# slimgroup/dfno

Hardware: AMD Instinct MI355X
Metric: sec/batch (lower is better)
Workload: dtype fp32; 1 GPU; model=dfno-two-phase-3d, global_batch=1, t_in=1, t_out=30, width=20, num_blocks=4, parallelism=spatial-model-parallel 1x1x1x1x1x1, step=fwd+relative-Lp-loss+bwd+adam, spectral_weights=complex64

## Files before the change

dfno_amd/csrc/adam.hip:

```cpp

#include <hip/hip_runtime.h>
#include <hip/hip_bf16.h>
#include <hip/hip_fp8.h>
#include <torch/extension.h>
#include <ATen/hip/impl/HIPStreamMasqueradingAsCUDA.h>

#include <map>
#include <vector>

#include "kernels.h"
#include "device_util.h"


namespace {

using namespace dfno_io;

constexpr int kBlock = 256;
constexpr long kGridCap = 256L * 8;

template <typename T, bool VECTOR>
__global__ void adam_step_kernel(T* __restrict__ p, const T* __restrict__ g,
                                 T* __restrict__ m, T* __restrict__ v,
                                 long n, T lr, T b1, T b2, T eps, T wd,
                                 T c1, T c2) {
  long i0 = (long)blockIdx.x * blockDim.x + threadIdx.x;
// ... 61 lines not shown
  for (long i = i0; i < total4; i += stride) {
    while (i >= tab.end4[t]) ++t;
    long base = (t == 0) ? 0 : tab.end4[t - 1];
    long j = (i - base) * 4;
    float4 pv = *reinterpret_cast<float4*>(tab.p[t] + j);
    const float4 gv = *reinterpret_cast<const float4*>(tab.g[t] + j);
    float4 mv = *reinterpret_cast<float4*>(tab.m[t] + j);
    float4 vv = *reinterpret_cast<float4*>(tab.v[t] + j);
    float pr[4] = {pv.x, pv.y, pv.z, pv.w};
    float gr[4] = {gv.x, gv.y, gv.z, gv.w};
    float mr[4] = {mv.x, mv.y, mv.z, mv.w};
    float vr[4] = {vv.x, vv.y, vv.z, vv.w};
    const float c1 = tab.c1[t], c2 = tab.c2[t];
#pragma unroll
    for (int k = 0; k < 4; ++k) {
      float gg = gr[k] + wd * pr[k];
      mr[k] = b1 * mr[k] + (1.f - b1) * gg;
      vr[k] = b2 * vr[k] + (1.f - b2) * gg * gg;
      pr[k] -= lr * (mr[k] / c1) / (sqrtf(vr[k] / c2) + eps);
    }
    *reinterpret_cast<float4*>(tab.p[t] + j) = make_float4(pr[0], pr[1], pr[2], pr[3]);
    *reinterpret_cast<float4*>(tab.m[t] + j) = make_float4(mr[0], mr[1], mr[2], mr[3]);
    *reinterpret_cast<float4*>(tab.v[t] + j) = make_float4(vr[0], vr[1], vr[2], vr[3]);
  }
}

struct AdamTabB {
  unsigned short* p[kAdamMaxT];
  const unsigned short* g[kAdamMaxT];
  unsigned short* m[kAdamMaxT];
  unsigned short* v[kAdamMaxT];
  long end8[kAdamMaxT];
  long nn[kAdamMaxT];
  float c1[kAdamMaxT], c2[kAdamMaxT];
// ... 7 lines not shown
  long stride = (long)gridDim.x * blockDim.x;
  int t = 0;
  for (long i = i0; i < total8; i += stride) {
    while (i >= tab.end8[t]) ++t;
    long base = (t == 0) ? 0 : tab.end8[t - 1];
    long j = (i - base) * 8;
    const float c1 = tab.c1[t], c2 = tab.c2[t];
    if (j + 8 <= tab.nn[t]) {
      float pr[8], gr[8], mr[8], vr[8];
      load8(tab.p[t] + j, pr);
      load8(tab.g[t] + j, gr);
      load8(tab.m[t] + j, mr);
      load8(tab.v[t] + j, vr);
#pragma unroll
      for (int k = 0; k < 8; ++k) {
        float gg = gr[k] + wd * pr[k];
        mr[k] = b1 * mr[k] + (1.f - b1) * gg;
        vr[k] = b2 * vr[k] + (1.f - b2) * gg * gg;
        pr[k] -= lr * (mr[k] / c1) / (sqrtf(vr[k] / c2) + eps);
      }
      store8(tab.p[t] + j, pr);
      store8(tab.m[t] + j, mr);
      store8(tab.v[t] + j, vr);
    } else {
      for (long e = j; e < tab.nn[t]; ++e) {
        float pv = __uint_as_float(((unsigned int)tab.p[t][e]) << 16);
        float gv = __uint_as_float(((unsigned int)tab.g[t][e]) << 16);
        float mv = __uint_as_float(((unsigned int)tab.m[t][e]) << 16);
        float vv = __uint_as_float(((unsigned int)tab.v[t][e]) << 16);
        float gg = gv + wd * pv;
        mv = b1 * mv + (1.f - b1) * gg;
        vv = b2 * vv + (1.f - b2) * gg * gg;
        pv -= lr * (mv / c1) / (sqrtf(vv / c2) + eps);
        __hip_bfloat16 hp = __float2bfloat16(pv);
        __hip_bfloat16 hm = __float2bfloat16(mv);
        __hip_bfloat16 hv = __float2bfloat16(vv);
        tab.p[t][e] = *reinterpret_cast<unsigned short*>(&hp);
        tab.m[t][e] = *reinterpret_cast<unsigned short*>(&hm);
        tab.v[t][e] = *reinterpret_cast<unsigned short*>(&hv);
      }
    }
  }
}

template <bool QOUT>
__global__ __launch_bounds__(kBlock) void adam_multi_uniform_kernel(
    AdamTab tab, AdamFp8Tab qt, long n4, float lr, float b1, float b2,
    float eps, float wd) {
// ... 7 lines not shown
  if constexpr (QOUT) inv = 448.f / fmaxf(*qt.am_in[t], 1e-30f);
  long i0 = (long)blockIdx.x * blockDim.x + threadIdx.x;
  long stride = (long)gridDim.x * blockDim.x;
  for (long i = i0; i < n4; i += stride) {
    long j = i * 4;
    float4 pv = *reinterpret_cast<float4*>(p + j);
    const float4 gv = *reinterpret_cast<const float4*>(g + j);
    float4 mv = *reinterpret_cast<float4*>(m + j);
    float4 vv = *reinterpret_cast<float4*>(v + j);
    float pr[4] = {pv.x, pv.y, pv.z, pv.w};
    float gr[4] = {gv.x, gv.y, gv.z, gv.w};
    float mr[4] = {mv.x, mv.y, mv.z, mv.w};
    float vr[4] = {vv.x, vv.y, vv.z, vv.w};
#pragma unroll
    for (int k = 0; k < 4; ++k) {
      float gg = gr[k] + wd * pr[k];
      mr[k] = b1 * mr[k] + (1.f - b1) * gg;
      vr[k] = b2 * vr[k] + (1.f - b2) * gg * gg;
      pr[k] -= lr * (mr[k] / c1) / (sqrtf(vr[k] / c2) + eps);
    }
    *reinterpret_cast<float4*>(p + j) = make_float4(pr[0], pr[1], pr[2], pr[3]);
    *reinterpret_cast<float4*>(m + j) = make_float4(mr[0], mr[1], mr[2], mr[3]);
    *reinterpret_cast<float4*>(v + j) = make_float4(vr[0], vr[1], vr[2], vr[3]);
    if constexpr (QOUT) {
      uchar4 qb;
      __hip_fp8_e4m3 h0(pr[0] * inv), h1(pr[1] * inv), h2(pr[2] * inv),
          h3(pr[3] * inv);
      qb.x = h0.__x; qb.y = h1.__x; qb.z = h2.__x; qb.w = h3.__x;
      *reinterpret_cast<uchar4*>(qt.q[t] + j) = qb;
#pragma unroll
      for (int k = 0; k < 4; ++k) amax = fmaxf(amax, fabsf(pr[k]));
    }
  }
  if constexpr (QOUT) {
// ... 204 lines not shown
```

dfno_amd/csrc/bindings.cpp:

```cpp
#include <torch/extension.h>

#include "kernels.h"

PYBIND11_MODULE(TORCH_EXTENSION_NAME, m) {
  m.doc() = "dfno_amd MI355X (gfx950) native kernels";
  m.def("channel_mix_fwd", &channel_mix_fwd,
        "fused channel linear + bias + gelu: returns (y, z)");
  m.def("channel_mix_fwd_t", &channel_mix_fwd_t,
        "transposed channel contraction (grad-x)");
  m.def("channel_mix_bwd_w", &channel_mix_bwd_w,
        "split-s grad-W (+grad-bias) reduction");
  m.def("linear_res_gelu_fwd", &linear_res_gelu_fwd,
        "fused y = gelu(W @ x + res): returns (y, z)");
  m.def("wide_channel_mix", &wide_channel_mix,
        "MFMA channel mix for 33 <= max(I, O) <= 128 (+bias/res/gelu, "
        "optionally transposed): returns (y, z)");
  m.def("irfft_linear_res_gelu_fwd", &irfft_linear_res_gelu_fwd,
        "fused y = gelu(W @ x + pad_irfft(Yt)): returns (y, z)");
  m.def("rfft_adj_mix", &rfft_adj_mix,
        "fused gx = W^T @ gz + rfft_trunc_adj(G, n)");
  m.def("gelu_fwd", &gelu_fwd, "exact gelu");
  m.def("gelu_bwd", &gelu_bwd, "gelu backward (gy, z) -> gz");
  m.def("add_gelu_fwd", &add_gelu_fwd, "fused residual add + gelu: returns (y, z)");
  m.def("proj_head_fwd", &proj_head_fwd, "fused linear->gelu->linear head");
// ... 25 lines not shown
        "fused padded (z,t) 2-D synthesis (kept-mode c64 -> real)");
  m.def("dft_pad_irfft_bf16", &dft_pad_irfft_bf16,
        "pad_irfft with bf16 output (bf16 compute config)");
  m.def("dft_rfft_trunc_adj_bf16", &dft_rfft_trunc_adj_bf16,
        "rfft_trunc adjoint with bf16 output");
  m.def("spectral_corner_fwd", &spectral_corner_fwd,
        "corner-block complex spectral contraction (accumulate into y box)");
  m.def("spectral_corner_bwd_x", &spectral_corner_bwd_x,
        "corner-block spectral contraction adjoint wrt x");
  m.def("spectral_corners_fwd", &spectral_corners_fwd,
        "all corner boxes in one launch");
  m.def("spectral_corners_bwd_x", &spectral_corners_bwd_x,
        "all corner boxes adjoint wrt x in one launch");
  m.def("spectral_corners_bwd_w", &spectral_corners_bwd_w,
        "multi-corner spectral grad-W (gw[i,o,e] = sum_b x conj(gy))");
  m.def("spectral_corners_fwd_fp8", &spectral_corners_fwd_fp8,
        "fp8-weight spectral contraction (e4m3 packed pairs + per-corner scale)");
  m.def("spectral_corners_bwd_x_fp8", &spectral_corners_bwd_x_fp8,
        "fp8-weight spectral contraction adjoint wrt x");
  m.def("fp8_quant_corners", &fp8_quant_corners,
        "device-side e4m3 requantization of the corner masters");
  m.def("bf16_channel_mix", &bf16_channel_mix,
        "bf16-storage fused channel linear (+bias/res/gelu): returns (y, z)");
  m.def("bf16_channel_mix_bwd_w", &bf16_channel_mix_bwd_w,
        "bf16 grad-W/grad-bias reduction (fp32 accumulation)");
  m.def("bf16_gelu_fwd", &bf16_gelu_fwd, "bf16 exact gelu");
  m.def("bf16_gelu_bwd", &bf16_gelu_bwd, "bf16 gelu backward");
  m.def("bf16_add_gelu", &bf16_add_gelu, "bf16 fused add+gelu: returns (y, z)");
  m.def("pack_boxes", &pack_boxes,
        "gather repartition boxes into one flat staging buffer");
// ... 4 lines not shown
```

dfno_amd/csrc/kernels.h:

```cpp
#pragma once

#include <torch/extension.h>
#define DFNO_CHECK_LAUNCH(what)                                            \
  do {                                                                     \
    hipError_t _e = hipGetLastError();                                     \
    TORCH_CHECK(_e == hipSuccess, what, " launch failed: ",                \
                hipGetErrorString(_e));                                    \
  } while (0)

#include <vector>

std::vector<at::Tensor> channel_mix_fwd(const at::Tensor& x, const at::Tensor& W,
                                        const at::Tensor& b, bool act);

at::Tensor channel_mix_fwd_t(const at::Tensor& gz, const at::Tensor& W);

std::vector<at::Tensor> linear_res_gelu_fwd(const at::Tensor& x, const at::Tensor& W,
                                            const at::Tensor& res);

std::vector<at::Tensor> wide_channel_mix(const at::Tensor& x, const at::Tensor& W,
                                         const at::Tensor& b, const at::Tensor& res,
                                         bool act, bool wt, bool need_z);

std::vector<at::Tensor> irfft_linear_res_gelu_fwd(const at::Tensor& x,
// ... 88 lines not shown
void unpack_boxes(const at::Tensor& flat, at::Tensor& dst,
                  const at::Tensor& desc, int64_t max_numel);

void spectral_corner_fwd(const at::Tensor& x, const at::Tensor& w, at::Tensor& y,
                         std::vector<int64_t> starts);
void spectral_corner_bwd_x(const at::Tensor& gy, const at::Tensor& w, at::Tensor& gx,
                           std::vector<int64_t> starts);

void spectral_corners_fwd(const at::Tensor& x, std::vector<at::Tensor> ws,
                          at::Tensor& y, std::vector<std::vector<int64_t>> starts);
void spectral_corners_bwd_x(const at::Tensor& gy, std::vector<at::Tensor> ws,
                            at::Tensor& gx, std::vector<std::vector<int64_t>> starts);
void spectral_corners_bwd_w(const at::Tensor& x, const at::Tensor& gy,
                            std::vector<at::Tensor> gws,
                            std::vector<std::vector<int64_t>> starts);

void spectral_corners_fwd_fp8(const at::Tensor& x, std::vector<at::Tensor> w16s,
                              std::vector<at::Tensor> amaxes, at::Tensor& y,
                              std::vector<std::vector<int64_t>> starts);
void spectral_corners_bwd_x_fp8(const at::Tensor& gy, std::vector<at::Tensor> w16s,
                                std::vector<at::Tensor> amaxes, at::Tensor& gx,
                                std::vector<std::vector<int64_t>> starts);
void fp8_quant_corners(std::vector<at::Tensor> ws, std::vector<at::Tensor> w16s,
                       std::vector<at::Tensor> amaxes);
```

dfno_amd/csrc/spectral.hip:

```cpp

#include <hip/hip_runtime.h>
#include <hip/hip_fp8.h>
#include <torch/extension.h>
#include <ATen/hip/impl/HIPStreamMasqueradingAsCUDA.h>

#include "kernels.h"
#include "device_util.h"

namespace {

using namespace dfno_io;

constexpr int kBlock = 256;
constexpr int kMaxDims = 6;

struct BoxGeom {
  long box[kMaxDims];
  long fstride[kMaxDims];
  long origin;
  int nd;
  long nelem;
};

template <typename T>
// ... 185 lines not shown
    } else {
      for (int i = 0; i < n_in; ++i) chan(i);
    }

    T* yb = y + 2 * (((long)b * n_out + o0) * Ftot + f);
#pragma unroll
    for (int k = 0; k < OTILE; ++k) {
      if (k < olim) {
        yb[2 * (long)k * Ftot] = accr[k];
        yb[2 * (long)k * Ftot + 1] = acci[k];
      }
    }
  }
}

template <typename T, int ICAP, bool ITILE = false>
__global__ __launch_bounds__(kBlock) void spectral_corners_bwd_w_kernel(
    const T* __restrict__ x, const T* __restrict__ gy, MultiGeom<T> mg,
    int B, int I_, int O, long Ftot) {
  const int ntile = ITILE ? (I_ + ICAP - 1) / ICAP : 1;
  const long total = mg.cum[mg.ncorners] * O * ntile;
  long t0 = (long)blockIdx.x * blockDim.x + threadIdx.x;
  long stride = (long)gridDim.x * blockDim.x;

  for (long t = t0; t < total; t += stride) {
    long work = t % mg.cum[mg.ncorners];
    int o = (int)(t / mg.cum[mg.ncorners]);
    int i0 = 0;
    if (ITILE) { i0 = (o / O) * ICAP; o %= O; }
    const int I = ITILE ? min(ICAP, I_ - i0) : I_;
// ... 15 lines not shown
      for (int k = 0; k < ICAP; ++k) {
        if (k < I) {
          const T xr = xb[2 * (long)k * Ftot], xi = xb[2 * (long)k * Ftot + 1];
          accr[k] += xr * gr + xi * gi;
          acci[k] += xr * gi - xi * gr;
        }
      }
    }
#pragma unroll
    for (int k = 0; k < ICAP; ++k) {
      if (k < I) {
        long widx = 2 * (((long)(i0 + k) * O + o) * g.nelem + e);
        gw[widx] = accr[k];
        gw[widx + 1] = acci[k];
      }
    }
  }
}


BoxGeom make_geom(const at::Tensor& x, const at::Tensor& w,
                  const std::vector<int64_t>& starts) {
  BoxGeom g{};
  int nd = (int)x.dim() - 2;
  TORCH_CHECK(nd >= 1 && nd <= kMaxDims, "spectral: bad ndim");
  TORCH_CHECK((int)w.dim() - 2 == nd, "spectral: w ndim mismatch");
  TORCH_CHECK((int)starts.size() == nd, "spectral: starts size mismatch");
  g.nd = nd;
  g.nelem = 1;
  long stride = 1;
  long fs[kMaxDims];
  for (int d = nd - 1; d >= 0; --d) {
    fs[d] = stride;
    stride *= x.size(d + 2);
  }
  g.origin = 0;
  for (int d = 0; d < nd; ++d) {
    g.box[d] = w.size(d + 2);
    g.fstride[d] = fs[d];
    g.origin += starts[d] * fs[d];
    g.nelem *= g.box[d];
  }
  return g;
}

void check_c(const at::Tensor& t, const char* name) {
  TORCH_CHECK(t.is_cuda(), name, " must be on GPU");
  TORCH_CHECK(t.is_contiguous(), name, " must be contiguous");
  TORCH_CHECK(t.scalar_type() == at::kComplexFloat || t.scalar_type() == at::kComplexDouble,
              name, " must be complex64/complex128");
}

}

void spectral_corner_fwd(const at::Tensor& x, const at::Tensor& w, at::Tensor& y,
                         std::vector<int64_t> starts) {
  check_c(x, "x"); check_c(w, "w"); check_c(y, "y");
  int B = (int)x.size(0), I = (int)x.size(1), O = (int)y.size(1);
  TORCH_CHECK((int)w.size(0) == I && (int)w.size(1) == O, "spectral: w shape");
  long Ftot = 1;
// ... 87 lines not shown
  for (long i = (long)blockIdx.x * blockDim.x + threadIdx.x; i < n;
       i += (long)gridDim.x * blockDim.x) {
    __hip_fp8_e4m3 h(src[i] * inv);
    dst[i] = h.__x;
  }
}

template <typename T, bool CONJT, bool FP8 = false>
static void launch_corners(const at::Tensor& x,
                           const std::vector<at::Tensor>& ws,
                           at::Tensor& y,
                           const std::vector<std::vector<int64_t>>& starts,
                           int B, int I, int O, long Ftot,
                           const std::vector<at::Tensor>* amaxes = nullptr) {
  auto stream = at::hip::getCurrentHIPStreamMasqueradingAsCUDA().stream();
  constexpr int OT = 8;
  const int n_out = CONJT ? I : O;
  long ntiles = (n_out + OT - 1) / OT;

  size_t idx = 0;
  while (idx < ws.size()) {
    MultiGeom<T> mg{};
    mg.ncorners = 0;
    mg.cum[0] = 0;
    while (idx < ws.size() && mg.ncorners < kMaxCorners) {
      BoxGeom g = make_geom(x, ws[idx], starts[idx]);
      if (g.nelem == 0) { ++idx; continue; }
      int c = mg.ncorners++;
      mg.g[c] = g;
      mg.w[c] = reinterpret_cast<const T*>(ws[idx].data_ptr());
      mg.amax[c] = amaxes ? (*amaxes)[idx].data_ptr<float>() : nullptr;
      mg.cum[c + 1] = mg.cum[c] + g.nelem * ntiles;
      ++idx;
    }
    if (mg.ncorners == 0) continue;
    int grid = launch_grid(mg.cum[mg.ncorners] * B, kBlock, 256L * 16);
    const int n_in = CONJT ? O : I;
#define SPC_LAUNCH(NINV)                                                       \
    hipLaunchKernelGGL((spectral_corners_kernel<T, OT, CONJT, NINV, FP8>),     \
                       dim3(grid), dim3(kBlock), 0, stream,                    \
                       reinterpret_cast<const T*>(x.data_ptr()), mg,           \
                       reinterpret_cast<T*>(y.data_ptr()), B, I, O, Ftot);
    if (n_in == 20) { SPC_LAUNCH(20) }
    else if (n_in == 32) { SPC_LAUNCH(32) }
    else if (n_in == 8) { SPC_LAUNCH(8) }
    else { SPC_LAUNCH(0) }
#undef SPC_LAUNCH
  }
}

void spectral_corners_fwd(const at::Tensor& x, std::vector<at::Tensor> ws,
                          at::Tensor& y, std::vector<std::vector<int64_t>> starts) {
// ... 162 lines not shown
  int B = (int)gy.size(0), O = (int)gy.size(1), I = (int)gx.size(1);
  long Ftot = 1;
  for (int d = 2; d < gy.dim(); ++d) Ftot *= gy.size(d);
  for (auto& w : ws) {
    check_c(w, "w");
    TORCH_CHECK((int)w.size(0) == I && (int)w.size(1) == O, "spectral: w shape");
  }
  if (B == 0 || ws.empty()) return;
  if (gy.scalar_type() == at::kComplexFloat) {
    launch_corners<float, true>(gy, ws, gx, starts, B, I, O, Ftot);
  } else {
    launch_corners<double, true>(gy, ws, gx, starts, B, I, O, Ftot);
  }
  DFNO_CHECK_LAUNCH("spectral");
}
```

dfno_amd/nn/block.py:

```python

from __future__ import annotations

import os
from typing import Dict, List, Tuple

import numpy as np
import torch
import torch.nn as nn

from ..comm import (Repartition, _get_plan, repartition_complete,
                    repartition_issue)
from ..partition import Partition, compute_distribution_info
from ..ops import spectral_conv, linear_res_gelu, rfft_trunc, fft_trunc, pad_ifft, pad_irfft
from ..ops import block_epilogue, fused_epilogue_enabled, fused_epilogue_ok
from ..ops.fft import (new_stash_key, rfft_bf16_native_ok, rfft_trunc_stash,
                       stash_fusable, zt_caps_ok, zt_enabled, zt_fwd, zt_inv,
                       zt_native_ok)
from ..timing import comm_region
from .linear import BroadcastedLinear

__all__ = ["DistributedFNOBlock"]


class DistributedFNOBlock(nn.Module):

    def __init__(self, P_x: Partition, in_shape, modes,
                 device=torch.device("cpu"), dtype=torch.float32,
                 spectral_fp8: bool = False):
# ... 70 lines not shown
                if digit == "0":
                    bounds.append((max(0, start) - start, min(mode, stop) - start))
                    gbounds.append((0, mode))
                else:
                    bounds.append((max(dim_size - mode, start) - start,
                                   min(dim_size, stop) - start))
                    gbounds.append((dim_size - mode, dim_size))
            bounds = list(reversed(bounds))
            gbounds = list(reversed(gbounds))
            if any(b - a <= 0 for a, b in bounds):
                continue
            w = nn.Parameter(
                self.scale * torch.rand(self.width, self.width,
                                        *[b - a for a, b in bounds],
                                        device=device, dtype=self.dtype_complex))
            self.weights.append(w)
            self.corner_bounds.append(bounds)
            self.slices.append([slice(None), slice(None)] + [slice(a, b) for a, b in bounds])
            self.corner_ids.append(i)
            self.corner_shapes.append([hi - lo for lo, hi in gbounds])
            loc = []
            for d, (glo, ghi) in zip(range(2, self.P_y.dim), gbounds):
                start, stop = info["start"][d], info["stop"][d]
                loc.append((max(start, glo) - glo, min(stop, ghi) - glo))
            self.corner_local_in_corner.append(loc)

        self.linear = BroadcastedLinear(self.P_x, self.width, self.width,
                                        bias=False, dim=1, device=device, dtype=dtype)

        self.dt_comm = 0.0
# ... 293 lines not shown
```

dfno_amd/ops/spectral.py:

```python

from __future__ import annotations

from typing import List, Sequence, Tuple

import torch

from .. import _ext

__all__ = ["spectral_conv"]


def _corner_slices(bounds: Sequence[Tuple[int, int]]):
    return (slice(None), slice(None)) + tuple(slice(a, b) for a, b in bounds)



_E4M3_MAX = 448.0
_QUANT_EPOCH = [0]
_FP8_CACHE = {}


def bump_quant_epoch() -> None:
    _QUANT_EPOCH[0] += 1
    if _QUANT_EPOCH[0] % 64 == 0:
# ... 25 lines not shown
        for i in range(0, len(stale), 64):
            ext.fp8_quant_corners(stale[i:i + 64], stale16[i:i + 64],
                                  stale_am[i:i + 64])
    out16 = [_FP8_CACHE[id(w)][1] for w in weights]
    amaxes = [_FP8_CACHE[id(w)][2] for w in weights]
    return out16, amaxes


def dequantize_fp8(w16: torch.Tensor, amax) -> torch.Tensor:
    if isinstance(amax, torch.Tensor):
        scale = float(amax.clamp_min(1e-30)) / _E4M3_MAX
    else:
        scale = float(amax)
    w8 = w16.unsqueeze(-1).view(torch.uint8).view(torch.float8_e4m3fn)
    return torch.view_as_complex(w8.to(torch.float32) * scale)


class _SpectralConvFn(torch.autograd.Function):
    @staticmethod
    def forward(ctx, x: torch.Tensor, bounds_list, out_channels: int,
                fp8: bool, *weights: torch.Tensor):
        B, I = x.shape[0], x.shape[1]
        fdims = list(x.shape[2:])
        ctx.fp8 = fp8 = bool(fp8 and x.is_cuda and x.dtype == torch.complex64)
        y = torch.zeros((B, out_channels, *fdims), dtype=x.dtype, device=x.device)
        if fp8 and x.numel() > 0:
            ext = _ext.get(required=True)
            xc = x.contiguous()
            w16s, scales = _fp8_weights(weights)
            ext.spectral_corners_fwd_fp8(
# ... 6 lines not shown
            xc = x.contiguous()
            ext.spectral_corners_fwd(
                xc, [w.contiguous() for w in weights], y,
                [[a for a, _ in bounds] for bounds in bounds_list])
            x_saved = xc
        else:
            if x.is_cuda and x.numel() > 0:
                from ..dispatch import note_fallback
                note_fallback("spectral_conv", f"dtype {x.dtype} not complex64/128")
            x_saved = x
            for w, bounds in zip(weights, bounds_list):
                sl = _corner_slices(bounds)
                y[sl] = torch.einsum("bi...,io...->bo...", x[sl], w)
        ctx.save_for_backward(x_saved, *weights)
        ctx.bounds_list = bounds_list
        return y

    @staticmethod
    def backward(ctx, gy: torch.Tensor):
        x = ctx.saved_tensors[0]
        weights = ctx.saved_tensors[1:]
        bounds_list = ctx.bounds_list
        gy = gy.contiguous()
        gx = torch.zeros_like(x)
        gws = []
        if gy.is_cuda and gy.numel() > 0 and gy.dtype in (torch.complex64, torch.complex128):
            ext = _ext.get(required=True)
            starts = [[a for a, _ in bounds] for bounds in bounds_list]
            if getattr(ctx, "fp8", False):
                w16s, scales = ctx.fp8_wq
                ext.spectral_corners_bwd_x_fp8(gy, w16s, scales, gx, starts)
            else:
                ext.spectral_corners_bwd_x(
                    gy, [w.contiguous() for w in weights], gx, starts)
            if x.shape[1] <= 64:
                gws = [torch.empty_like(w) for w in weights]
                ext.spectral_corners_bwd_w(x.contiguous(), gy, gws, starts)
            else:
                from ..dispatch import note_fallback
                note_fallback("spectral_corners_bwd_w",
                              f"in_channels {x.shape[1]} > 64 (einsum grad-W)")
                for w, bounds in zip(weights, bounds_list):
                    sl = _corner_slices(bounds)
                    gws.append(torch.einsum("bo...,bi...->io...",
                                            gy[sl], x[sl].conj()))
        else:
            for w, bounds in zip(weights, bounds_list):
                sl = _corner_slices(bounds)
                gx[sl] = torch.einsum("bo...,io...->bi...", gy[sl], w.conj())
                gws.append(torch.einsum("bo...,bi...->io...", gy[sl], x[sl].conj()))
        return (gx, None, None, None, *gws)


def spectral_conv(x: torch.Tensor, weights: List[torch.Tensor],
                  bounds_list: List[List[Tuple[int, int]]],
                  out_channels: int = None, fp8: bool = False) -> torch.Tensor:
    if out_channels is None:
        out_channels = weights[0].shape[1] if weights else x.shape[1]
    return _SpectralConvFn.apply(x, bounds_list, out_channels, fp8, *weights)
```

dfno_amd/optim.py:

```python

from __future__ import annotations

import torch

from . import _ext

__all__ = ["Adam"]


class Adam(torch.optim.Adam):

    def __init__(self, *args, **kwargs):
        super().__init__(*args, **kwargs)
        self._flat_cache = {}

    def _flat_views(self, p, state):
        def flat(t):
            r = torch.view_as_real(t) if t.is_complex() else t
            assert r.is_contiguous(), "fused Adam requires contiguous params"
            return r.view(-1)
        ptrs = (p.data_ptr(), state["exp_avg"].data_ptr(),
                state["exp_avg_sq"].data_ptr())
        cached = self._flat_cache.get(id(p))
        if cached is None or cached[0] != ptrs:
            cached = (ptrs, (flat(p), flat(state["exp_avg"]),
                             flat(state["exp_avg_sq"])))
            self._flat_cache[id(p)] = cached
        return cached[1]

    @torch.no_grad()
    def step(self, closure=None):
        loss = None
        if closure is not None:
            with torch.enable_grad():
                loss = closure()

        ext = _ext.get(required=False) if torch.cuda.is_available() else None
        fallback_groups = []
        for group in self.param_groups:
            lr = group["lr"]
            beta1, beta2 = group["betas"]
            eps = group["eps"]
            wd = group["weight_decay"]
            if group.get("amsgrad", False) or ext is None:
                fallback_groups.append(group)
                continue
            slow = []
            batch = ([], [], [], [], [])
            fp8_q, fp8_in, fp8_out, origs = [], [], [], []
            try:
                from .ops.spectral import _FP8_CACHE, _QUANT_EPOCH
            except Exception:
# ... 66 lines not shown
```

training/two_phase/train_two_phase.py:

```python

import argparse
import os
import sys
import time
from pathlib import Path

import numpy as np
import torch

sys.path.insert(0, str(Path(__file__).resolve().parents[2]))

import dfno_amd as dfno
from dfno_amd.data import DistributedSleipnerDataset3D


def main():
    p = argparse.ArgumentParser()
    p.add_argument("--ranks", "-n", type=int, default=None,
                   help="partition size along Y (default: world size)")
    p.add_argument("--data", choices=["synthetic", "local", "azure"], default="synthetic")
    p.add_argument("--data-root", type=str, default=None)
    p.add_argument("--num-train", type=int, default=800)
    p.add_argument("--num-valid", type=int, default=200)
    p.add_argument("--num-epochs", type=int, default=100)
# ... 49 lines not shown
    valid_idx = list(range(args.num_train + 1, args.num_train + args.num_valid + 1))
    mk = lambda idx: DistributedSleipnerDataset3D(
        P_x, idx, client=client, container=container, prefix=prefix,
        shape=shape, normalize=True, savepath=args.cache_dir,
        filename="sample", root=root, synthetic=synthetic)
    train_data, valid_data = mk(train_idx), mk(valid_idx)

    train_loader = torch.utils.data.DataLoader(train_data, batch_size=nb, shuffle=False)
    valid_loader = torch.utils.data.DataLoader(valid_data, batch_size=nb, shuffle=False)
    P_x.barrier()

    model = dfno.DistributedFNONd(
        P_x, [nb, channel_in, *shape[:-1], 1], shape[-1], args.width,
        tuple(args.modes), device=device, dtype=dtype)
    criterion = dfno.DistributedRelativeLpLoss(P_x)
    optimizer = torch.optim.Adam(model.parameters(), lr=args.lr)

    out_dir = Path(args.out_dir)
    if P_root.active:
        out_dir.mkdir(parents=True, exist_ok=True)
    train_accs, valid_accs = [], []

    start_epoch = 0
    if args.resume:
        rdir = Path(args.resume)
        rk = max(P_x.rank, 0)
        cands = sorted(rdir.glob(f"train_state_*_{rk:04d}.pt"))
        if not cands:
            raise FileNotFoundError(
                f"rank {rk}: no train_state_*_{rk:04d}.pt under {rdir}")
        state = torch.load(cands[-1], map_location=device, weights_only=False)
# ... 89 lines not shown
```

Measured before the change: 18.40 ms.

## Fuse spectral grad-W into Adam update and add paired-element spectral contraction kernel

Adds a kernel that computes the spectral corner weight gradient and applies Adam to those weights in the same pass. This is done by deferring grad-W from backward to the optimizer step, so the gradient tensors are never written or read back. It also adds a paired-element spectral contraction path (two frequencies per thread, float4 loads, 4-wide output tiles) for fp32 corners, which can be disabled with an env var. The training script switches to the custom Adam, and the Adam maths moves into a shared helper. The deferral logic brings extra bookkeeping complexity and fallback paths, and it changes when gradients exist.

```diff
diff --git a/dfno_amd/csrc/adam.hip b/dfno_amd/csrc/adam.hip
--- a/dfno_amd/csrc/adam.hip
+++ b/dfno_amd/csrc/adam.hip
@@ -10,6 +10,7 @@
 
 #include "kernels.h"
 #include "device_util.h"
+#include "adam_update.h"
 
 
 namespace {
@@ -101,10 +102,7 @@
     const float c1 = tab.c1[t], c2 = tab.c2[t];
 #pragma unroll
     for (int k = 0; k < 4; ++k) {
-      float gg = gr[k] + wd * pr[k];
-      mr[k] = b1 * mr[k] + (1.f - b1) * gg;
-      vr[k] = b2 * vr[k] + (1.f - b2) * gg * gg;
-      pr[k] -= lr * (mr[k] / c1) / (sqrtf(vr[k] / c2) + eps);
+      adam_update(pr[k], gr[k], mr[k], vr[k], lr, b1, b2, eps, wd, c1, c2);
     }
     *reinterpret_cast<float4*>(tab.p[t] + j) = make_float4(pr[0], pr[1], pr[2], pr[3]);
     *reinterpret_cast<float4*>(tab.m[t] + j) = make_float4(mr[0], mr[1], mr[2], mr[3]);
@@ -142,10 +140,7 @@
       load8(tab.v[t] + j, vr);
 #pragma unroll
       for (int k = 0; k < 8; ++k) {
-        float gg = gr[k] + wd * pr[k];
-        mr[k] = b1 * mr[k] + (1.f - b1) * gg;
-        vr[k] = b2 * vr[k] + (1.f - b2) * gg * gg;
-        pr[k] -= lr * (mr[k] / c1) / (sqrtf(vr[k] / c2) + eps);
+        adam_update(pr[k], gr[k], mr[k], vr[k], lr, b1, b2, eps, wd, c1, c2);
       }
       store8(tab.p[t] + j, pr);
       store8(tab.m[t] + j, mr);
@@ -156,10 +151,7 @@
         float gv = __uint_as_float(((unsigned int)tab.g[t][e]) << 16);
         float mv = __uint_as_float(((unsigned int)tab.m[t][e]) << 16);
         float vv = __uint_as_float(((unsigned int)tab.v[t][e]) << 16);
-        float gg = gv + wd * pv;
-        mv = b1 * mv + (1.f - b1) * gg;
-        vv = b2 * vv + (1.f - b2) * gg * gg;
-        pv -= lr * (mv / c1) / (sqrtf(vv / c2) + eps);
+        adam_update(pv, gv, mv, vv, lr, b1, b2, eps, wd, c1, c2);
         __hip_bfloat16 hp = __float2bfloat16(pv);
         __hip_bfloat16 hm = __float2bfloat16(mv);
         __hip_bfloat16 hv = __float2bfloat16(vv);
@@ -197,10 +189,7 @@
     float vr[4] = {vv.x, vv.y, vv.z, vv.w};
 #pragma unroll
     for (int k = 0; k < 4; ++k) {
-      float gg = gr[k] + wd * pr[k];
-      mr[k] = b1 * mr[k] + (1.f - b1) * gg;
-      vr[k] = b2 * vr[k] + (1.f - b2) * gg * gg;
-      pr[k] -= lr * (mr[k] / c1) / (sqrtf(vr[k] / c2) + eps);
+      adam_update(pr[k], gr[k], mr[k], vr[k], lr, b1, b2, eps, wd, c1, c2);
     }
     *reinterpret_cast<float4*>(p + j) = make_float4(pr[0], pr[1], pr[2], pr[3]);
     *reinterpret_cast<float4*>(m + j) = make_float4(mr[0], mr[1], mr[2], mr[3]);
diff --git a/dfno_amd/csrc/adam_update.h b/dfno_amd/csrc/adam_update.h
--- /dev/null
+++ b/dfno_amd/csrc/adam_update.h
@@ -0,0 +1,13 @@
+#pragma once
+
+#include <hip/hip_runtime.h>
+
+__device__ __forceinline__ void adam_update(float& p, float g, float& m,
+                                            float& v, float lr, float b1,
+                                            float b2, float eps, float wd,
+                                            float c1, float c2) {
+  float gg = g + wd * p;
+  m = b1 * m + (1.f - b1) * gg;
+  v = b2 * v + (1.f - b2) * gg * gg;
+  p -= lr * (m / c1) / (sqrtf(v / c2) + eps);
+}
diff --git a/dfno_amd/csrc/bindings.cpp b/dfno_amd/csrc/bindings.cpp
--- a/dfno_amd/csrc/bindings.cpp
+++ b/dfno_amd/csrc/bindings.cpp
@@ -63,6 +63,8 @@
         "all corner boxes adjoint wrt x in one launch");
   m.def("spectral_corners_bwd_w", &spectral_corners_bwd_w,
         "multi-corner spectral grad-W (gw[i,o,e] = sum_b x conj(gy))");
+  m.def("spectral_gradw_adam_", &spectral_gradw_adam_,
+        "spectral grad-W fused into the Adam update of the corner weights");
   m.def("spectral_corners_fwd_fp8", &spectral_corners_fwd_fp8,
         "fp8-weight spectral contraction (e4m3 packed pairs + per-corner scale)");
   m.def("spectral_corners_bwd_x_fp8", &spectral_corners_bwd_x_fp8,
diff --git a/dfno_amd/csrc/kernels.h b/dfno_amd/csrc/kernels.h
--- a/dfno_amd/csrc/kernels.h
+++ b/dfno_amd/csrc/kernels.h
@@ -126,6 +126,13 @@
 void spectral_corners_bwd_w(const at::Tensor& x, const at::Tensor& gy,
                             std::vector<at::Tensor> gws,
                             std::vector<std::vector<int64_t>> starts);
+void spectral_gradw_adam_(const at::Tensor& x, const at::Tensor& gy,
+                          std::vector<at::Tensor> ps,
+                          std::vector<at::Tensor> ms,
+                          std::vector<at::Tensor> vs,
+                          std::vector<std::vector<int64_t>> starts,
+                          double lr, double beta1, double beta2, double eps,
+                          double weight_decay, std::vector<int64_t> steps);
 
 void spectral_corners_fwd_fp8(const at::Tensor& x, std::vector<at::Tensor> w16s,
                               std::vector<at::Tensor> amaxes, at::Tensor& y,
diff --git a/dfno_amd/csrc/spectral.hip b/dfno_amd/csrc/spectral.hip
--- a/dfno_amd/csrc/spectral.hip
+++ b/dfno_amd/csrc/spectral.hip
@@ -4,8 +4,11 @@
 #include <torch/extension.h>
 #include <ATen/hip/impl/HIPStreamMasqueradingAsCUDA.h>
 
+#include <cstdlib>
+
 #include "kernels.h"
 #include "device_util.h"
+#include "adam_update.h"
 
 namespace {
 
@@ -223,6 +226,72 @@
   }
 }
 
+template <int OTILE, bool CONJT, int NIN = 0>
+__global__ __launch_bounds__(kBlock) void spectral_corners_pair_kernel(
+    const float* __restrict__ x, MultiGeom<float> mg, float* __restrict__ y,
+    int B, int I, int O, long Ftot) {
+  const int n_out = CONJT ? I : O;
+  const int n_in = NIN > 0 ? NIN : (CONJT ? O : I);
+  const long total = mg.cum[mg.ncorners] * B;
+
+  long t0 = (long)blockIdx.x * blockDim.x + threadIdx.x;
+  long stride = (long)gridDim.x * blockDim.x;
+
+  for (long t = t0; t < total; t += stride) {
+    long work = t % mg.cum[mg.ncorners];
+    int b = (int)(t / mg.cum[mg.ncorners]);
+    int c = 0;
+    while (work >= mg.cum[c + 1]) ++c;
+    work -= mg.cum[c];
+    const BoxGeom& g = mg.g[c];
+    const float* w = mg.w[c];
+    const long npair = g.nelem / 2;
+    const long e = (work % npair) * 2;
+    const int tile = (int)(work / npair);
+
+    const long f = box_to_global(e, g);
+    const int o0 = tile * OTILE;
+    const int olim = min(OTILE, n_out - o0);
+
+    float4 acc[OTILE];
+#pragma unroll
+    for (int k = 0; k < OTILE; ++k) acc[k] = make_float4(0.f, 0.f, 0.f, 0.f);
+
+    const float* xb = x + 2 * (((long)b * n_in) * Ftot + f);
+    auto chan = [&](int i) {
+      const float4 xv = *reinterpret_cast<const float4*>(xb + 2 * (long)i * Ftot);
+#pragma unroll
+      for (int k = 0; k < OTILE; ++k) {
+        if (k < olim) {
+          const long pidx = CONJT
+              ? (((long)(o0 + k)) * O + i) * g.nelem + e
+              : ((long)i * O + o0 + k) * g.nelem + e;
+          const float4 wv = *reinterpret_cast<const float4*>(w + 2 * pidx);
+          if (CONJT) {
+            cmac_conj(acc[k].x, acc[k].y, wv.x, wv.y, xv.x, xv.y);
+            cmac_conj(acc[k].z, acc[k].w, wv.z, wv.w, xv.z, xv.w);
+          } else {
+            cmac(acc[k].x, acc[k].y, xv.x, xv.y, wv.x, wv.y);
+            cmac(acc[k].z, acc[k].w, xv.z, xv.w, wv.z, wv.w);
+          }
+        }
+      }
+    };
+    if constexpr (NIN > 0) {
+#pragma unroll
+      for (int i = 0; i < NIN; ++i) chan(i);
+    } else {
+      for (int i = 0; i < n_in; ++i) chan(i);
+    }
+
+    float* yb = y + 2 * (((long)b * n_out + o0) * Ftot + f);
+#pragma unroll
+    for (int k = 0; k < OTILE; ++k) {
+      if (k < olim) *reinterpret_cast<float4*>(yb + 2 * (long)k * Ftot) = acc[k];
+    }
+  }
+}
+
 template <typename T, int ICAP, bool ITILE = false>
 __global__ __launch_bounds__(kBlock) void spectral_corners_bwd_w_kernel(
     const T* __restrict__ x, const T* __restrict__ gy, MultiGeom<T> mg,
@@ -268,6 +337,107 @@
         gw[widx] = accr[k];
         gw[widx + 1] = acci[k];
       }
+    }
+  }
+}
+
+struct GradwAdamTab {
+  BoxGeom g[kMaxCorners];
+  float* p[kMaxCorners];
+  float* m[kMaxCorners];
+  float* v[kMaxCorners];
+  float c1[kMaxCorners], c2[kMaxCorners];
+  long cum[kMaxCorners + 1];
+  int ncorners;
+};
+
+template <int EPT>
+__device__ __forceinline__ void ldc(const float* p, float* out) {
+  if constexpr (EPT == 2) {
+    const float4 t = *reinterpret_cast<const float4*>(p);
+    out[0] = t.x; out[1] = t.y; out[2] = t.z; out[3] = t.w;
+  } else {
+    const float2 t = *reinterpret_cast<const float2*>(p);
+    out[0] = t.x; out[1] = t.y;
+  }
+}
+
+template <int EPT>
+__device__ __forceinline__ void stc(float* p, const float* v) {
+  if constexpr (EPT == 2) {
+    *reinterpret_cast<float4*>(p) = make_float4(v[0], v[1], v[2], v[3]);
+  } else {
+    *reinterpret_cast<float2*>(p) = make_float2(v[0], v[1]);
+  }
+}
+
+template <int NI, int EPT>
+__global__ __launch_bounds__(kBlock) void spectral_gradw_adam_kernel(
+    const float* __restrict__ x, const float* __restrict__ gy,
+    GradwAdamTab tab, int B, int I_, int O, long Ftot, float lr, float b1,
+    float b2, float eps, float wd) {
+  const int I = NI > 0 ? NI : I_;
+  const long total = tab.cum[tab.ncorners] * O;
+  long t0 = (long)blockIdx.x * blockDim.x + threadIdx.x;
+  long stride = (long)gridDim.x * blockDim.x;
+
+  for (long t = t0; t < total; t += stride) {
+    long work = t % tab.cum[tab.ncorners];
+    const int o = (int)(t / tab.cum[tab.ncorners]);
+    int c = 0;
+    while (work >= tab.cum[c + 1]) ++c;
+    const long e = (work - tab.cum[c]) * EPT;
+    const BoxGeom& g = tab.g[c];
+    float* __restrict__ p = tab.p[c];
+    float* __restrict__ m = tab.m[c];
+    float* __restrict__ v = tab.v[c];
+    const float c1 = tab.c1[c], c2 = tab.c2[c];
+
+    const long f = box_to_global(e, g);
+    const float* gy0 = gy + 2 * ((long)o * Ftot + f);
+    const float* x0 = x + 2 * f;
+    float gv0[2 * EPT];
+    ldc<EPT>(gy0, gv0);
+
+    auto chan = [&](int i) {
+      float acc[2 * EPT];
+#pragma unroll
+      for (int k = 0; k < 2 * EPT; ++k) acc[k] = 0.f;
+      for (int b = 0; b < B; ++b) {
+        float gv[2 * EPT], xv[2 * EPT];
+        if (b == 0) {
+#pragma unroll
+          for (int k = 0; k < 2 * EPT; ++k) gv[k] = gv0[k];
+        } else {
+          ldc<EPT>(gy0 + 2 * (long)b * O * Ftot, gv);
+        }
+        ldc<EPT>(x0 + 2 * ((long)b * I + i) * Ftot, xv);
+#pragma unroll
+        for (int k = 0; k < EPT; ++k) {
+          const float xr = xv[2 * k], xi = xv[2 * k + 1];
+          const float gr = gv[2 * k], gi = gv[2 * k + 1];
+          acc[2 * k] += xr * gr + xi * gi;
+          acc[2 * k + 1] += xr * gi - xi * gr;
+        }
+      }
+      const long widx = 2 * (((long)i * O + o) * g.nelem + e);
+      float pr[2 * EPT], mr[2 * EPT], vr[2 * EPT];
+      ldc<EPT>(p + widx, pr);
+      ldc<EPT>(m + widx, mr);
+      ldc<EPT>(v + widx, vr);
+#pragma unroll
+      for (int k = 0; k < 2 * EPT; ++k)
+        adam_update(pr[k], acc[k], mr[k], vr[k], lr, b1, b2, eps, wd, c1, c2);
+      stc<EPT>(p + widx, pr);
+      stc<EPT>(m + widx, mr);
+      stc<EPT>(v + widx, vr);
+    };
+    if constexpr (NI > 0) {
+#pragma unroll
+      for (int i = 0; i < NI; ++i) chan(i);
+    } else {
+#pragma unroll 4
+      for (int i = 0; i < I; ++i) chan(i);
     }
   }
 }
@@ -298,6 +468,13 @@
   return g;
 }
 
+bool pair_ok(const at::Tensor& spec, const at::Tensor& w,
+             const std::vector<int64_t>& starts) {
+  const int64_t last = spec.dim() - 1;
+  return aligned16(w.data_ptr()) && w.size(last) % 2 == 0 &&
+         spec.size(last) % 2 == 0 && starts.back() % 2 == 0;
+}
+
 void check_c(const at::Tensor& t, const char* name) {
   TORCH_CHECK(t.is_cuda(), name, " must be on GPU");
   TORCH_CHECK(t.is_contiguous(), name, " must be contiguous");
@@ -415,8 +592,53 @@
                            int B, int I, int O, long Ftot,
                            const std::vector<at::Tensor>* amaxes = nullptr) {
   auto stream = at::hip::getCurrentHIPStreamMasqueradingAsCUDA().stream();
+  const int n_out = CONJT ? I : O;
+  const int n_in = CONJT ? O : I;
+
+  if constexpr (std::is_same<T, float>::value && !FP8) {
+    const char* env = std::getenv("DFNO_SPECTRAL_PAIR");
+    bool pair = !(env && env[0] == '0') && aligned16(x.data_ptr()) &&
+                aligned16(y.data_ptr());
+    for (size_t k = 0; pair && k < ws.size(); ++k)
+      pair = ws[k].dim() == x.dim() &&
+             (int64_t)starts[k].size() == x.dim() - 2 &&
+             (ws[k].numel() == 0 || pair_ok(x, ws[k], starts[k]));
+    constexpr int ot = 4;
+    if (pair) {
+      size_t idx = 0;
+      while (idx < ws.size()) {
+        MultiGeom<float> mg{};
+        mg.ncorners = 0;
+        mg.cum[0] = 0;
+        const long ntiles = (n_out + ot - 1) / ot;
+        while (idx < ws.size() && mg.ncorners < kMaxCorners) {
+          BoxGeom g = make_geom(x, ws[idx], starts[idx]);
+          if (g.nelem == 0) { ++idx; continue; }
+          int c = mg.ncorners++;
+          mg.g[c] = g;
+          mg.w[c] = reinterpret_cast<const float*>(ws[idx].data_ptr());
+          mg.cum[c + 1] = mg.cum[c] + (g.nelem / 2) * ntiles;
+          ++idx;
+        }
+        if (mg.ncorners == 0) continue;
+        int grid = launch_grid(mg.cum[mg.ncorners] * B, kBlock, 256L * 16);
+#define SPP_LAUNCH(NINV)                                                       \
+        hipLaunchKernelGGL((spectral_corners_pair_kernel<ot, CONJT, NINV>),    \
+                           dim3(grid), dim3(kBlock), 0, stream,                \
+                           reinterpret_cast<const float*>(x.data_ptr()), mg,   \
+                           reinterpret_cast<float*>(y.data_ptr()), B, I, O,    \
+                           Ftot);
+        if (n_in == 20) { SPP_LAUNCH(20) }
+        else if (n_in == 32) { SPP_LAUNCH(32) }
+        else if (n_in == 8) { SPP_LAUNCH(8) }
+        else { SPP_LAUNCH(0) }
+#undef SPP_LAUNCH
+      }
+      return;
+    }
+  }
+
   constexpr int OT = 8;
-  const int n_out = CONJT ? I : O;
   long ntiles = (n_out + OT - 1) / OT;
 
   size_t idx = 0;
@@ -436,7 +658,6 @@
     }
     if (mg.ncorners == 0) continue;
     int grid = launch_grid(mg.cum[mg.ncorners] * B, kBlock, 256L * 16);
-    const int n_in = CONJT ? O : I;
 #define SPC_LAUNCH(NINV)                                                       \
     hipLaunchKernelGGL((spectral_corners_kernel<T, OT, CONJT, NINV, FP8>),     \
                        dim3(grid), dim3(kBlock), 0, stream,                    \
@@ -629,3 +850,89 @@
   }
   DFNO_CHECK_LAUNCH("spectral");
 }
+
+void spectral_gradw_adam_(const at::Tensor& x, const at::Tensor& gy,
+                          std::vector<at::Tensor> ps,
+                          std::vector<at::Tensor> ms,
+                          std::vector<at::Tensor> vs,
+                          std::vector<std::vector<int64_t>> starts,
+                          double lr, double beta1, double beta2, double eps,
+                          double weight_decay, std::vector<int64_t> steps) {
+  check_c(x, "x"); check_c(gy, "gy");
+  TORCH_CHECK(x.scalar_type() == at::kComplexFloat &&
+              gy.scalar_type() == at::kComplexFloat,
+              "spectral_gradw_adam_: complex64 only");
+  const size_t n = ps.size();
+  TORCH_CHECK(ms.size() == n && vs.size() == n && starts.size() == n &&
+              steps.size() == n, "spectral_gradw_adam_: list size mismatch");
+  TORCH_CHECK(x.dim() == gy.dim() && x.size(0) == gy.size(0),
+              "spectral_gradw_adam_: x/gy shape mismatch");
+  const int nd = (int)x.dim() - 2;
+  for (int d = 0; d < nd; ++d)
+    TORCH_CHECK(x.size(d + 2) == gy.size(d + 2),
+                "spectral_gradw_adam_: x/gy shape mismatch");
+  int B = (int)x.size(0), I = (int)x.size(1), O = (int)gy.size(1);
+  long Ftot = 1;
+  for (int d = 2; d < x.dim(); ++d) Ftot *= x.size(d);
+  if (B == 0 || n == 0 || I == 0 || O == 0) return;
+
+  bool vec = aligned16(x.data_ptr()) && aligned16(gy.data_ptr());
+  for (size_t k = 0; k < n; ++k) {
+    const at::Tensor& p = ps[k];
+    check_c(p, "p"); check_c(ms[k], "exp_avg"); check_c(vs[k], "exp_avg_sq");
+    TORCH_CHECK(p.scalar_type() == at::kComplexFloat &&
+                ms[k].scalar_type() == at::kComplexFloat &&
+                vs[k].scalar_type() == at::kComplexFloat,
+                "spectral_gradw_adam_: complex64 only");
+    TORCH_CHECK(p.dim() == x.dim() && (int)p.size(0) == I &&
+                (int)p.size(1) == O, "spectral_gradw_adam_: p shape");
+    TORCH_CHECK(ms[k].sizes() == p.sizes() && vs[k].sizes() == p.sizes(),
+                "spectral_gradw_adam_: state shape");
+    TORCH_CHECK((int)starts[k].size() == nd, "spectral_gradw_adam_: starts");
+    for (int d = 0; d < nd; ++d)
+      TORCH_CHECK(starts[k][d] >= 0 &&
+                  starts[k][d] + p.size(d + 2) <= x.size(d + 2),
+                  "spectral_gradw_adam_: corner box outside the spectrum");
+    vec = vec && pair_ok(x, p, starts[k]) && aligned16(ms[k].data_ptr()) &&
+          aligned16(vs[k].data_ptr());
+  }
+
+  auto stream = at::hip::getCurrentHIPStreamMasqueradingAsCUDA().stream();
+  const int ept = vec ? 2 : 1;
+  size_t idx = 0;
+  while (idx < n) {
+    GradwAdamTab tab{};
+    tab.ncorners = 0;
+    tab.cum[0] = 0;
+    while (idx < n && tab.ncorners < kMaxCorners) {
+      BoxGeom g = make_geom(x, ps[idx], starts[idx]);
+      if (g.nelem == 0) { ++idx; continue; }
+      int c = tab.ncorners++;
+      tab.g[c] = g;
+      tab.p[c] = reinterpret_cast<float*>(ps[idx].data_ptr());
+      tab.m[c] = reinterpret_cast<float*>(ms[idx].data_ptr());
+      tab.v[c] = reinterpret_cast<float*>(vs[idx].data_ptr());
+      tab.c1[c] = (float)(1.0 - std::pow(beta1, (double)steps[idx]));
+      tab.c2[c] = (float)(1.0 - std::pow(beta2, (double)steps[idx]));
+      tab.cum[c + 1] = tab.cum[c] + g.nelem / ept;
+      ++idx;
+    }
+    if (tab.ncorners == 0) continue;
+    int grid = launch_grid(tab.cum[tab.ncorners] * O, kBlock, 256L * 32);
+#define SGA_LAUNCH(NI_, EPT_)                                                  \
+    hipLaunchKernelGGL((spectral_gradw_adam_kernel<NI_, EPT_>), dim3(grid),    \
+                       dim3(kBlock), 0, stream,                                \
+                       reinterpret_cast<const float*>(x.data_ptr()),           \
+                       reinterpret_cast<const float*>(gy.data_ptr()), tab, B,  \
+                       I, O, Ftot, (float)lr, (float)beta1, (float)beta2,      \
+                       (float)eps, (float)weight_decay);
+#define SGA_EPT(NI_) if (vec) { SGA_LAUNCH(NI_, 2) } else { SGA_LAUNCH(NI_, 1) }
+    if (I == 20) { SGA_EPT(20) }
+    else if (I == 32) { SGA_EPT(32) }
+    else if (I == 8) { SGA_EPT(8) }
+    else { SGA_EPT(0) }
+#undef SGA_EPT
+#undef SGA_LAUNCH
+  }
+  DFNO_CHECK_LAUNCH("spectral_gradw_adam");
+}
diff --git a/dfno_amd/nn/block.py b/dfno_amd/nn/block.py
--- a/dfno_amd/nn/block.py
+++ b/dfno_amd/nn/block.py
@@ -12,6 +12,7 @@
                     repartition_issue)
 from ..partition import Partition, compute_distribution_info
 from ..ops import spectral_conv, linear_res_gelu, rfft_trunc, fft_trunc, pad_ifft, pad_irfft
+from ..ops.spectral import CORNER_TAG
 from ..ops import block_epilogue, fused_epilogue_enabled, fused_epilogue_ok
 from ..ops.fft import (new_stash_key, rfft_bf16_native_ok, rfft_trunc_stash,
                        stash_fusable, zt_caps_ok, zt_enabled, zt_fwd, zt_inv,
@@ -112,6 +113,7 @@
                 self.scale * torch.rand(self.width, self.width,
                                         *[b - a for a, b in bounds],
                                         device=device, dtype=self.dtype_complex))
+            setattr(w, CORNER_TAG, True)
             self.weights.append(w)
             self.corner_bounds.append(bounds)
             self.slices.append([slice(None), slice(None)] + [slice(a, b) for a, b in bounds])
diff --git a/dfno_amd/ops/spectral.py b/dfno_amd/ops/spectral.py
--- a/dfno_amd/ops/spectral.py
+++ b/dfno_amd/ops/spectral.py
@@ -1,6 +1,8 @@
 
 from __future__ import annotations
 
+import os
+import weakref
 from typing import List, Sequence, Tuple
 
 import torch
@@ -63,6 +65,54 @@
         scale = float(amax)
     w8 = w16.unsqueeze(-1).view(torch.uint8).view(torch.float8_e4m3fn)
     return torch.view_as_complex(w8.to(torch.float32) * scale)
+
+
+
+CORNER_TAG = "_dfno_spectral_corner"
+_CORNER_OWNER = {}
+
+
+def fused_spectral_adam_enabled() -> bool:
+    return os.environ.get("DFNO_FUSED_SPECTRAL_ADAM", "1") != "0"
+
+
+def register_corners(optimizer, params) -> None:
+    dead = [k for k, (wr, orf) in _CORNER_OWNER.items()
+            if wr() is None or orf() is None]
+    for k in dead:
+        del _CORNER_OWNER[k]
+    for p in params:
+        if getattr(p, CORNER_TAG, False) and p.dtype == torch.complex64:
+            _CORNER_OWNER[id(p)] = (weakref.ref(p), weakref.ref(optimizer))
+
+
+def _corner_owner(weights):
+    owner = None
+    for w in weights:
+        ent = _CORNER_OWNER.get(id(w))
+        if ent is None or ent[0]() is not w:
+            return None
+        opt = ent[1]()
+        if opt is None or (owner is not None and opt is not owner):
+            return None
+        owner = opt
+    return owner
+
+
+def corner_grads(x, gy, bounds_list, weights):
+    if (gy.is_cuda and gy.numel() > 0 and x.shape[1] <= 64
+            and gy.dtype in (torch.complex64, torch.complex128)):
+        ext = _ext.get(required=True)
+        gws = [torch.empty_like(w) for w in weights]
+        ext.spectral_corners_bwd_w(
+            x.contiguous(), gy, gws,
+            [[a for a, _ in bounds] for bounds in bounds_list])
+        return gws
+    gws = []
+    for w, bounds in zip(weights, bounds_list):
+        sl = _corner_slices(bounds)
+        gws.append(torch.einsum("bo...,bi...->io...", gy[sl], x[sl].conj()))
+    return gws
 
 
 class _SpectralConvFn(torch.autograd.Function):
@@ -99,7 +149,33 @@
                 y[sl] = torch.einsum("bi...,io...->bo...", x[sl], w)
         ctx.save_for_backward(x_saved, *weights)
         ctx.bounds_list = bounds_list
+        ctx.corner_params = (
+            weights if weights and not fp8 and x.dtype == torch.complex64
+            and _corner_owner(weights) is not None else None)
         return y
+
+    @staticmethod
+    def _deferral_owner(ctx, x):
+        params = ctx.corner_params
+        if params is None or not fused_spectral_adam_enabled():
+            return None
+        if torch.is_grad_enabled() or x.shape[1] > 64:
+            return None
+        if not all(ctx.needs_input_grad[4:]):
+            return None
+        opt = _corner_owner(params)
+        if opt is None:
+            return None
+        if opt.has_pending(params):
+            opt.materialize_grads()
+            return None
+        for w in params:
+            ent = _FP8_CACHE.get(id(w))
+            if w.grad is not None or (ent is not None
+                                      and ent[1].shape == w.shape
+                                      and ent[1].device == w.device):
+                return None
+        return opt if opt.accepts_deferred(params) else None
 
     @staticmethod
     def backward(ctx, gy: torch.Tensor):
@@ -109,6 +185,9 @@
         gy = gy.contiguous()
         gx = torch.zeros_like(x)
         gws = []
+        owner = _SpectralConvFn._deferral_owner(ctx, x)
+        if owner is not None:
+            gws = [None] * len(weights)
         if gy.is_cuda and gy.numel() > 0 and gy.dtype in (torch.complex64, torch.complex128):
             ext = _ext.get(required=True)
             starts = [[a for a, _ in bounds] for bounds in bounds_list]
@@ -118,22 +197,20 @@
             else:
                 ext.spectral_corners_bwd_x(
                     gy, [w.contiguous() for w in weights], gx, starts)
-            if x.shape[1] <= 64:
-                gws = [torch.empty_like(w) for w in weights]
-                ext.spectral_corners_bwd_w(x.contiguous(), gy, gws, starts)
-            else:
-                from ..dispatch import note_fallback
-                note_fallback("spectral_corners_bwd_w",
-                              f"in_channels {x.shape[1]} > 64 (einsum grad-W)")
-                for w, bounds in zip(weights, bounds_list):
-                    sl = _corner_slices(bounds)
-                    gws.append(torch.einsum("bo...,bi...->io...",
-                                            gy[sl], x[sl].conj()))
+            if owner is None:
+                if x.shape[1] > 64:
+                    from ..dispatch import note_fallback
+                    note_fallback("spectral_corners_bwd_w",
+                                  f"in_channels {x.shape[1]} > 64 (einsum grad-W)")
+                gws = corner_grads(x, gy, bounds_list, weights)
         else:
             for w, bounds in zip(weights, bounds_list):
                 sl = _corner_slices(bounds)
                 gx[sl] = torch.einsum("bo...,io...->bi...", gy[sl], w.conj())
-                gws.append(torch.einsum("bo...,bi...->io...", gy[sl], x[sl].conj()))
+            if owner is None:
+                gws = corner_grads(x, gy, bounds_list, weights)
+        if owner is not None:
+            owner.add_pending(x, gy, bounds_list, ctx.corner_params)
         return (gx, None, None, None, *gws)
 
 
diff --git a/dfno_amd/optim.py b/dfno_amd/optim.py
--- a/dfno_amd/optim.py
+++ b/dfno_amd/optim.py
@@ -4,6 +4,7 @@
 import torch
 
 from . import _ext
+from .ops import spectral as _spectral
 
 __all__ = ["Adam"]
 
@@ -13,6 +14,80 @@
     def __init__(self, *args, **kwargs):
         super().__init__(*args, **kwargs)
         self._flat_cache = {}
+        self._pending = []
+        for group in self.param_groups:
+            _spectral.register_corners(self, group["params"])
+
+    def add_param_group(self, param_group):
+        super().add_param_group(param_group)
+        if hasattr(self, "_pending"):
+            _spectral.register_corners(self, self.param_groups[-1]["params"])
+
+    def _group_of(self, p):
+        for group in self.param_groups:
+            if any(q is p for q in group["params"]):
+                return group
+        return None
+
+    def accepts_deferred(self, weights) -> bool:
+        group = self._group_of(weights[0])
+        return (group is not None
+                and not group.get("amsgrad", False)
+                and not group.get("maximize", False)
+                and all(any(q is w for q in group["params"]) for w in weights))
+
+    def has_pending(self, weights) -> bool:
+        ids = {id(w) for w in weights}
+        return any(id(w) in ids for ent in self._pending for w in ent[3])
+
+    def add_pending(self, x, gy, bounds_list, weights) -> None:
+        self._pending.append((x, gy, bounds_list, tuple(weights)))
+
+    @torch.no_grad()
+    def materialize_grads(self) -> None:
+        pending, self._pending = self._pending, []
+        for x, gy, bounds_list, weights in pending:
+            for w, gw in zip(weights, _spectral.corner_grads(
+                    x, gy, bounds_list, weights)):
+                if w.grad is None:
+                    w.grad = gw
+                else:
+                    w.grad += gw
+
+    def zero_grad(self, set_to_none: bool = True):
+        self._pending = []
+        return super().zero_grad(set_to_none=set_to_none)
+
+    def _step_pending(self, ext) -> None:
+        pending, self._pending = self._pending, []
+        for ent in pending:
+            x, gy, bounds_list, weights = ent
+            group = self._group_of(weights[0])
+            if (not x.is_cuda or x.numel() == 0
+                    or any(w.grad is not None or not w.is_contiguous()
+                           for w in weights)):
+                self._pending = [ent]
+                self.materialize_grads()
+                continue
+            ms, vs, steps = [], [], []
+            for w in weights:
+                state = self.state[w]
+                if len(state) == 0:
+                    state["step"] = torch.tensor(0.0)
+                    state["exp_avg"] = torch.zeros_like(w)
+                    state["exp_avg_sq"] = torch.zeros_like(w)
+                state["step"] += 1
+                ms.append(state["exp_avg"])
+                vs.append(state["exp_avg_sq"])
+                steps.append(int(state["step"].item()))
+            beta1, beta2 = group["betas"]
+            for i in range(0, len(weights), 8):
+                ext.spectral_gradw_adam_(
+                    x, gy, [w.detach() for w in weights[i:i + 8]],
+                    ms[i:i + 8], vs[i:i + 8],
+                    [[a for a, _ in b] for b in bounds_list[i:i + 8]],
+                    group["lr"], beta1, beta2, group["eps"],
+                    group["weight_decay"], steps[i:i + 8])
 
     def _flat_views(self, p, state):
         def flat(t):
@@ -36,6 +111,11 @@
                 loss = closure()
 
         ext = _ext.get(required=False) if torch.cuda.is_available() else None
+        if self._pending:
+            if ext is None:
+                self.materialize_grads()
+            else:
+                self._step_pending(ext)
         fallback_groups = []
         for group in self.param_groups:
             lr = group["lr"]
diff --git a/training/two_phase/train_two_phase.py b/training/two_phase/train_two_phase.py
--- a/training/two_phase/train_two_phase.py
+++ b/training/two_phase/train_two_phase.py
@@ -87,7 +87,8 @@
         P_x, [nb, channel_in, *shape[:-1], 1], shape[-1], args.width,
         tuple(args.modes), device=device, dtype=dtype)
     criterion = dfno.DistributedRelativeLpLoss(P_x)
-    optimizer = torch.optim.Adam(model.parameters(), lr=args.lr)
+    from dfno_amd.optim import Adam
+    optimizer = Adam(model.parameters(), lr=args.lr)
 
     out_dir = Path(args.out_dir)
     if P_root.active:
```

New measurement: 17.26 ms (median of 6 runs). 1.07x faster.
